# entn-at/tf-kaldi-speaker

Hardware: AMD Instinct MI355X
Metric: utterances/sec x-vector extraction (30-dim x 300-frame) (higher is better)
Workload: dtype f16+fp6-cross(f32-split); 1 GPU; tdnn x-vector (tdnn6_dense), statistics_pooling, 256 utt/GPU/step of 300 frames x 30 dims; batch_per_gpu=256, frames=300, node=tdnn6_dense, precision=f16f6, parallelism=utterance-shard x1, launch=stream launches

## Files before the change

tf-kaldi-speaker_amd/csrc/api_forward.hip:

```cpp
#include "xv_model.h"

using namespace xv;
using namespace xv::api;

namespace {

struct Run {
  xv_handle* h;
  const xv_plan* p;
  const float* feats;
  int feat_ld;
  float* out;
  char* ws;
  hipStream_t s;
  int f16;
  int B;
  const int32_t* off;
  char* raw(int64_t o) const { return o >= 0 ? ws + o : nullptr; }
  float* f32(int64_t o) const { return reinterpret_cast<float*>(raw(o)); }
  const float* in(int64_t o) const { return o == -2 ? feats : f32(o); }
  float* dst(const PlanStep& st) const { return st.out_off >= 0 ? f32(st.out_off) : out; }
  int* ovf() const { return static_cast<int*>(h->ovf_flag.p); }
};

// ... 25 lines not shown
  GemmArgs a{};
  a.X = r.in(st.in0_off);
  a.ldx = op.in0 == 0 ? r.feat_ld : L.cin;
  a.cin = L.cin; a.M = st.M; a.K = L.K(); a.N = L.cout;
  a.Wt = static_cast<const float*>(L.wt.p); a.Kpad = L.Kpad; a.Npad = L.Npad;
  const bool bn_stage = st.stage >= ST_BN;
  a.scale = (bn_stage || !L.has_bn) ? L.d_scale() : L.d_ones();
  a.shift = (bn_stage || !L.has_bn) ? L.d_shift() : L.d_bias();
  a.act = (st.stage == ST_ACT) ? L.act : ACT_NONE;
  a.alpha = (a.act == ACT_PRELU) ? L.d_alpha() : nullptr;
  a.rowmap = st.rowmap >= 0 ? static_cast<const int32_t*>(r.p->d_rowmaps.p) + r.p->rowmap_off[st.rowmap] : nullptr;
  a.Y = r.dst(st); a.ldy = L.cout;
  a.f16 = r.f16;
  a.slab3 = h->opt_slab3;
  a.ovf = r.ovf();
  a.sb_mul = std::ldexp(1.f, L.out_exp);
  if (L.mode == 1 || L.mode == 2 || L.mode == 3) {
    const int64_t Sin = h->values[op.in0].grid_S;
    a.a_pitch = (L.mode == 3 ? Sin : L.sw) * (int64_t)L.cin;
    a.a_off = L.mode == 1 ? (L.sw == 1 ? 0 : L.cin) : (L.mode == 2 ? (Sin + 1) * L.cin : L.cin);
    if (st.compact()) {
      a.arow = static_cast<const int32_t*>(r.p->d_rowmaps.p) + r.p->rowmap_off[st.arow];
      a.a_pitch = L.cin;
      a.a_off = L.mode == 1 ? 0 : (Sin + 1) * L.cin;
    }
    a.ntaps = L.mode == 1 ? 3 : 1;
    a.ktap = L.mode == 1 ? 3 * L.cin : (L.mode == 2 ? L.cin : L.Fin * L.cin);
    a.tap_stride = Sin * L.cin;
    a.cin = a.K;
  }
  if (op.in1 > 0) { a.R = r.in(st.in1_off); a.ldr = L.cout; }
  if (st.fuse_att == 1) {
    a.Y = nullptr;
    a.att_part = r.f32(st.out_off);
    a.att_ld = st.att_ld;
    a.att_heads = d.att_num_heads;
    a.att_q = static_cast<const float*>(h->query_eff.p);
  } else if (st.fuse_att == 2) {
    a.Y = nullptr;
    a.pool_part = r.f32(st.out_off);
    a.pool_row2utt = static_cast<const int32_t*>(r.p->d_row2utt.p);
    a.pool_slotbase = static_cast<const int32_t*>(r.p->d_slotbase.p);
    a.pool_w = r.f32(st.att_w_off);
    a.pool_heads = d.att_num_heads;
    a.pool_split = d.att_split_value;
    a.pool_dvh = d.att_split_value ? L.cout / d.att_num_heads : L.cout;
    a.pool_odim = h->pool_dim / 2;
  }
  if (st.fuse_pool) {
    a.Y = nullptr;
    a.pool_part = r.f32(st.out_off);
    a.pool_row2utt = static_cast<const int32_t*>(r.p->d_row2utt.p);
    a.pool_slotbase = static_cast<const int32_t*>(r.p->d_slotbase.p);
  }
  if (st.out_sb_off >= 0) {
    a.Ysb = r.raw(st.out_sb_off);
    a.ldsb = sb_ld(L.cout);
    if (st.out_off < 0 && !st.to_out) a.Y = nullptr;
  }
  return a;
}

int gemm_clear_border(const Run& r, const PlanStep& st, const Layer& L, const Value& vo) {
  xv_handle* h = r.h;
  const size_t head = (size_t)vo.grid_S + 1;
  const size_t rows0 = st.grid_cover && L.mode != 4 ? head : (st.grid_cover ? 0 : (size_t)st.rows_out + vo.grid_S);
  if (st.compact() || st.trows()) {
    XV_HIP(h, launch_grid_zero_border(r.p->dev_offsets(st.lvl_out), r.B, st.frames_out, vo.grid_F, vo.grid_S, L.cout / 4,
                                      sb_ld(L.cout) / 4, r.f32(st.out_off), r.raw(st.out_sb_off), r.s));
  } else {
    if (rows0 > 0) {
      if (st.out_off >= 0) XV_HIP(h, hipMemsetAsync(r.raw(st.out_off), 0, rows0 * L.cout * 4, r.s));
      if (st.out_sb_off >= 0) XV_HIP(h, hipMemsetAsync(r.raw(st.out_sb_off), 0, rows0 * sb_ld(L.cout) * 4, r.s));
    }
    const size_t tail = 2 * (size_t)vo.grid_S + 2;
    if (tail > (size_t)kSlackRows) return fail(h, XV_ERR_STATE, "grid pitch %d: the window overreach does not fit the slack", vo.grid_S);
    if (st.out_off >= 0) XV_HIP(h, hipMemsetAsync(r.f32(st.out_off) + (size_t)st.rows_out * L.cout, 0, tail * L.cout * 4, r.s));
    if (st.out_sb_off >= 0)
      XV_HIP(h, hipMemsetAsync(static_cast<char*>(r.raw(st.out_sb_off)) + (size_t)st.rows_out * sb_ld(L.cout) * 4, 0,
                               tail * sb_ld(L.cout) * 4, r.s));
  }
  return XV_OK;
}

int launch_conv0(const Run& r, const PlanStep& st, const Layer& L, const Value& vo, GemmArgs& a) {
  xv_handle* h = r.h;
  if (st.scratch_off < 0) return fail(h, XV_ERR_STATE, "conv0 has no scratch");
  a.cin = 32; a.K = 32;
  const bool direct = L.use_split && !st.to_out && st.stage == L.final_stage() && L.cout % 8 == 0 &&
                      (st.out_sb_off < 0 || L.cout % 32 == 0) && L.cout <= 256 && L.wdir.p;
  if (direct) {
    XV_HIP(h, launch_conv0_direct(r.feats, r.feat_ld, r.off, r.B, L.Fout, vo.grid_S, L.cout, st.M, static_cast<const float*>(L.wdir.p),
                                  L.act, L.d_alpha(), r.f32(st.out_off), r.raw(st.out_sb_off), sb_ld(L.cout), r.f16, r.ovf(),
                                  a.sb_mul, r.s));
  } else if (L.use_split) {
    XV_HIP(h, launch_im2col2d_sb(r.feats, r.feat_ld, r.off, r.B, L.Fout, vo.grid_S, st.M, r.raw(st.scratch_off), r.f16, r.ovf(), r.s));
    a.Xsb = r.raw(st.scratch_off); a.ldsbx = 32; a.Wsb = L.wsb.p; a.Wfr = L.wfr.p;
    XV_HIP(h, launch_gemm_bf16x3(a, r.s));
  } else {
    XV_HIP(h, launch_im2col2d_f32(r.feats, r.feat_ld, r.off, r.B, L.Fout, vo.grid_S, st.M, r.f32(st.scratch_off), r.s));
    a.X = r.f32(st.scratch_off); a.ldx = 32;
    XV_HIP(h, launch_gemm_f32(a, true, r.s));
  }
  return XV_OK;
}

// ... 319 lines not shown
```

tf-kaldi-speaker_amd/csrc/api_plan.hip:

```cpp
#include "xv_arena.h"
#include "xv_model.h"

using namespace xv;
using namespace xv::api;

namespace {

constexpr size_t kPoolMaxBuffers = 96, kPoolMaxBytes = (size_t)1 << 30;

hipError_t pool_take(xv_handle* h, size_t bytes, DevBuf& out) {
  out = DevBuf();
  if (bytes == 0) return hipSuccess;
  {
    std::lock_guard<std::mutex> lk(h->pool_mu);
    int best = -1;
    for (size_t i = 0; i < h->pool.size(); ++i)
      if (h->pool[i].bytes >= bytes && h->pool[i].bytes <= 4 * bytes + 4096 &&
          (best < 0 || h->pool[i].bytes < h->pool[best].bytes))
        best = (int)i;
    if (best >= 0) {
      out = h->pool[best];
      h->pool_bytes -= out.bytes;
      h->pool.erase(h->pool.begin() + best);
      return hipSuccess;
// ... 33 lines not shown
  BatchShape& sh = *out;
  sh.B = batch;
  for (int b = 0; b < batch; ++b) {
    const int64_t len = (int64_t)frame_offsets[b + 1] - frame_offsets[b];
    if (len <= need_ctx)
      return fail(h, XV_ERR_TOO_SHORT, "utterance %d has %lld frames; node '%s' needs more than %d", b, (long long)len,
                  h->nodes[node_id].name.c_str(), need_ctx);
    if (len != (int64_t)frame_offsets[1] - frame_offsets[0]) sh.uniform = false;
  }
  const int64_t F0 = frame_offsets[batch];
  if (F0 > (int64_t)1 << 30) return fail(h, XV_ERR_INVALID, "batch of %lld frames is too large for 32-bit row indices", (long long)F0);
  for (const Value& v : h->values) sh.max_level = std::max(sh.max_level, v.tlevel);
  for (int64_t& f : sh.Fl) f = F0;
  sh.lvl[0].assign(frame_offsets, frame_offsets + batch + 1);
  for (int k = 1; k <= sh.max_level && k < 4; ++k) {
    sh.lvl[k].resize(batch + 1);
    sh.lvl[k][0] = 0;
    for (int b = 0; b < batch; ++b) sh.lvl[k][b + 1] = sh.lvl[k][b] + (sh.lvl[k - 1][b + 1] - sh.lvl[k - 1][b] + 1) / 2;
    sh.Fl[k] = sh.lvl[k][batch];
  }
  return XV_OK;
}

std::vector<int> producers(const xv_handle* h) {
  std::vector<int> producer(h->values.size(), -1);
  for (size_t i = 0; i < h->ops.size(); ++i) producer[h->ops[i].out] = (int)i;
  return producer;
}

std::vector<int> plan_order(const xv_handle* h, int target_op, const std::vector<int>& producer) {
  std::vector<char> need(h->ops.size(), 0);
  std::vector<int> stack{target_op};
  while (!stack.empty()) {
    const int o = stack.back();
    stack.pop_back();
    if (need[o]) continue;
    need[o] = 1;
    for (int in : {h->ops[o].in0, h->ops[o].in1})
      if (in > 0 && producer[in] >= 0) stack.push_back(producer[in]);
  }
  std::vector<int> order;
  for (size_t i = 0; i < h->ops.size(); ++i) if (need[i]) order.push_back((int)i);
  return order;
}

struct Fusion {
  int key_prod = -1;
  int val_prod = -1;
  int att_pool_value = -1;
  int fused_value = -1;
  int slot_value = -1;
  std::vector<int> order;
  std::vector<int32_t> slotbase;
  int64_t pool_slots = 0;
};

int readers_of(const xv_handle* h, const std::vector<int>& order, int v) {
  int n = 0;
  for (int o : order)
    if (h->ops[o].in0 == v || h->ops[o].in1 == v) ++n;
  return n;
}

int att_fusable(const xv_handle* h, const std::vector<int>& order, const std::vector<int>& producer, int target_op, int v) {
  if (v <= 0 || producer[v] < 0 || producer[v] == target_op) return -1;
  const Op& prod = h->ops[producer[v]];
  if (prod.kind != OP_GEMM || prod.in1 > 0 || readers_of(h, order, v) != 1) return -1;
  const Layer& L = h->layers[prod.layer];
  return (L.use_split && !L.im2col && L.mode == 0 && L.w == 1 && (L.cout & 3) == 0) ? producer[v] : -1;
}

Fusion plan_fusion(const xv_handle* h, int target_op, const std::vector<int>& producer, std::vector<int> order, const BatchShape& sh) {
  Fusion f;
  if (h->opt_att_fusion && h->desc.pooling_type == XV_POOL_SELF_ATTENTION && h->desc.att_num_heads <= 8) {
    int softmax_op = -1, pool_op = -1;
    for (int o : order) {
      if (h->ops[o].kind == OP_ATT_SCORES) f.key_prod = att_fusable(h, order, producer, target_op, h->ops[o].in0);
      if (h->ops[o].kind == OP_ATT_SOFTMAX) softmax_op = o;
      if (h->ops[o].kind == OP_ATT_POOL) pool_op = o;
    }
    if (pool_op >= 0 && softmax_op >= 0) {
      const int H = h->desc.att_num_heads, dv = h->att_dv;
      const bool heads_ok = H == 1 || !h->desc.att_split_value || (dv / H) % 32 == 0;
      const int vp = heads_ok ? att_fusable(h, order, producer, target_op, h->ops[pool_op].in0) : -1;
      if (vp >= 0) {
        f.val_prod = vp;
        f.att_pool_value = h->ops[pool_op].in0;
        order.erase(std::find(order.begin(), order.end(), vp));
        order.insert(std::find(order.begin(), order.end(), pool_op), vp);
      }
    }
  }
  for (int o : order) {
    const Op& op = h->ops[o];
    if (op.kind != OP_STAT_POOL || op.in0 <= 0 || producer[op.in0] < 0) continue;
    const Op& prod = h->ops[producer[op.in0]];
    if (prod.kind != OP_GEMM || producer[op.in0] == target_op) continue;
    const Layer& L = h->layers[prod.layer];
    if (readers_of(h, order, op.in0) == 1 && L.w == 1 && (L.cout & 3) == 0 && h->opt_pool_fusion) f.fused_value = op.in0;
  }
  f.slot_value = f.fused_value >= 0 ? f.fused_value : f.att_pool_value;
  if (f.slot_value >= 0) {
    const int ctx = h->values[f.slot_value].ctx;
    const std::vector<int32_t>& so = sh.lvl[h->values[f.slot_value].tlevel];
    f.slotbase.resize(sh.B);
    for (int b = 0; b < sh.B; ++b) {
      const int r0 = so[b] - b * ctx, r1 = so[b + 1] - (b + 1) * ctx;
      const int t0 = r0 >> 6, t1 = (r1 - 1) >> 6;
      f.slotbase[b] = (int32_t)(f.pool_slots - t0);
      f.pool_slots += t1 - t0 + 1;
    }
  }
  f.order = std::move(order);
  return f;
}

struct PlanCtx {
  const xv_handle* h;
  const Node& node;
  const BatchShape& sh;
  const Fusion& fu;
  int64_t rows(int v) const { return value_rows(h, v, sh.Fl, sh.B); }
};

struct RowMaps {
  std::vector<int64_t> off;
  int64_t elems = 0;
  int add(int64_t n) { off.push_back(elems); elems += n; return (int)off.size() - 1; }
};

struct Placement {
  Arena arena;
  std::vector<int64_t> off, size, off_sb, size_sb;
  std::vector<char> want_f32, want_sb;
  std::vector<int> last_use;
  void free_value(int v) {
    if (size[v] > 0) { arena.release(off[v], size[v]); size[v] = 0; }
    if (size_sb[v] > 0) { arena.release(off_sb[v], size_sb[v]); size_sb[v] = 0; }
  }
};

Placement make_placement(const xv_handle* h, const std::vector<int>& order) {
  const size_t nv = h->values.size();
  Placement pl;
  pl.off.assign(nv, -1); pl.off_sb.assign(nv, -1);
  pl.size.assign(nv, 0); pl.size_sb.assign(nv, 0);
  pl.want_f32.assign(nv, 0); pl.want_sb.assign(nv, 0);
  pl.last_use.assign(nv, -1);
  for (size_t s = 0; s < order.size(); ++s) {
    const Op& op = h->ops[order[s]];
    const bool split_in = op.kind == OP_GEMM && h->layers[op.layer].use_split;
    if (op.in0 > 0) (split_in ? pl.want_sb : pl.want_f32)[op.in0] = 1;
    if (op.in1 > 0) pl.want_f32[op.in1] = 1;
    for (int in : {op.in0, op.in1})
      if (in > 0) pl.last_use[in] = (int)s;
  }
  return pl;
}

void gemm_form(const PlanCtx& c, const Op& op, const Layer& L, PlanStep& st, RowMaps& rm) {
  const xv_handle* h = c.h;
  const int64_t padded_rows = c.sh.Fl[st.lvl_in] + 2 * (int64_t)c.sh.B;
  const bool grid = L.mode == 1 || L.mode == 2;
// ... 259 lines not shown
  const Layer& L = h->layers[op.layer];
  const int B = p->info.batch;
  const Value& vi = h->values[op.in0];
  const Value& vo = h->values[op.out];
  const int32_t* doff = p->dev_offsets(st.lvl_in);
  int32_t* maps = static_cast<int32_t*>(p->d_rowmaps.p);
  int32_t* rm = maps + p->rowmap_off[st.rowmap];
  switch (st.form) {
    case FORM_ROWS: return launch_build_rowmap(doff, B, vi.ctx, L.w, rm, st.M, s);
    case FORM_TROWS: return launch_build_rowmap_trows(doff, B, vo.grid_S, rm, st.M, s);
    case FORM_COMPACT:
      return launch_build_rowmap_grid_compact(doff, p->dev_offsets(st.lvl_out), B, vi.grid_S, vo.grid_S, L.Fout, L.sw, L.st,
                                              L.mode == 1 ? 3 : 1, maps + p->rowmap_off[st.arow], rm, st.M, align_up(st.M, 128), s);
    case FORM_GRID:
      if (L.st == 2)
        return launch_build_rowmap_grid_ts(doff, p->dev_offsets(st.lvl_out), B, vi.grid_S / L.sw, L.Fout, vo.grid_S,
                                           L.mode == 1 ? 3 : 1, rm, st.M, s);
      return launch_build_rowmap_grid(doff, B, vi.grid_S / L.sw, L.Fout, vo.grid_S, st.grid_cover ? 1 : 0, rm, st.M, s);
    case FORM_CONV5: return launch_build_rowmap_rows(doff, B, rm, st.M, s);
    default: return launch_build_rowmap_interior(doff, B, L.Fout, vo.grid_S, rm, st.M, s);
  }
}

hipError_t upload_index_arrays(xv_plan* p, const BatchShape& sh, int64_t rowmap_elems, int slot_value, hipStream_t s, const char** what) {
  xv_handle* h = p->h;
  const size_t nb = (size_t)(sh.B + 1) * 4;
  hipError_t e = hipSuccess;
  DeviceGuard g(h->device);
  *what = "hipMalloc(offsets)";
  if ((e = pool_take(h, nb, p->d_offsets)) != hipSuccess) return e;
  *what = "hipMemcpyAsync(offsets)";
  if ((e = hipMemcpyAsync(p->d_offsets.p, p->lvl_offsets[0].data(), nb, hipMemcpyHostToDevice, s)) != hipSuccess) return e;
  for (int k = 1; k <= sh.max_level && k < 4; ++k) {
    *what = "hipMalloc(level offsets)";
    if ((e = pool_take(h, nb, p->d_lvl[k])) != hipSuccess) return e;
    *what = "hipMemcpyAsync(level offsets)";
    if ((e = hipMemcpyAsync(p->d_lvl[k].p, p->lvl_offsets[k].data(), nb, hipMemcpyHostToDevice, s)) != hipSuccess) return e;
  }
  if (rowmap_elems > 0) {
    *what = "hipMalloc(rowmaps)";
    if ((e = pool_take(h, (size_t)rowmap_elems * 4, p->d_rowmaps)) != hipSuccess) return e;
    *what = "build_rowmap";
    for (const PlanStep& st : p->steps)
      if (st.rowmap >= 0 && (e = build_rowmap(p, st, s)) != hipSuccess) return e;
  }
  if (slot_value >= 0) {
    const int64_t rows = value_rows(h, slot_value, sh.Fl, sh.B);
    *what = "hipMalloc(row2utt)";
    if ((e = pool_take(h, (size_t)rows * 4, p->d_row2utt)) != hipSuccess) return e;
    *what = "hipMalloc(slotbase)";
    if ((e = pool_take(h, (size_t)sh.B * 4, p->d_slotbase)) != hipSuccess) return e;
    *what = "hipMemcpyAsync(slotbase)";
    if ((e = hipMemcpyAsync(p->d_slotbase.p, p->offsets_slotbase.data(), (size_t)sh.B * 4, hipMemcpyHostToDevice, s)) != hipSuccess) return e;
    *what = "build_row2utt";
    e = launch_build_row2utt(p->dev_offsets(h->values[slot_value].tlevel), sh.B, h->values[slot_value].ctx,
                             static_cast<int32_t*>(p->d_row2utt.p), (int)rows, s);
  }
  return e;
}

}

extern "C" {

int xv_plan_create(xv_handle* h, const int32_t* frame_offsets, int batch, int node_id, void* stream, xv_plan** out) {
  if (!h) return fail(nullptr, XV_ERR_INVALID, "xv_plan_create: null handle");
  if (!out || !frame_offsets) return fail(h, XV_ERR_INVALID, "xv_plan_create: null argument");
  *out = nullptr;
  if (!h->finalized) return fail(h, XV_ERR_STATE, "xv_plan_create before xv_finalize");
  if (batch < 1) return fail(h, XV_ERR_INVALID, "xv_plan_create: batch %d < 1", batch);
  if (node_id < 0 || node_id >= (int)h->nodes.size()) return fail(h, XV_ERR_INVALID, "xv_plan_create: bad node id %d", node_id);
  const Node& node = h->nodes[node_id];
  BatchShape sh;
  if (const int rc = plan_shape(h, frame_offsets, batch, node_id, &sh)) return rc;
  if (node.att_weights && !sh.uniform)
    return fail(h, XV_ERR_INVALID, "attention_weights [b,h,l] needs utterances of equal length");
  const std::vector<int> producer = producers(h);
  const Fusion fu = plan_fusion(h, node.op, producer, plan_order(h, node.op, producer), sh);

  xv_plan* p = new (std::nothrow) xv_plan();
  if (!p) return fail(h, XV_ERR_HIP, "out of host memory");
  p->h = h;
  for (int k = 0; k <= sh.max_level && k < 4; ++k) p->lvl_offsets[k] = sh.lvl[k];
  p->pool_slots = fu.pool_slots;
  p->offsets_slotbase = fu.slotbase;

  const PlanCtx ctx{h, node, sh, fu};
  Placement pl = make_placement(h, fu.order);
  RowMaps rm;
  int64_t total_flops = 0;
  for (size_t s = 0; s < fu.order.size(); ++s) {
    p->steps.push_back(plan_step(ctx, s, p->steps, pl, rm));
    total_flops += p->steps.back().flops;
  }
  p->rowmap_off = rm.off;
  for (size_t i = 0; i < p->steps.size(); ++i)
    if (p->steps[i].flops > p->steps[p->dominant_step].flops) p->dominant_step = (int)i;
  chain_two_unit(h, p->steps);
  p->info = plan_output_info(h, node_id, sh, total_flops, pl.arena.top());

  const char* what = "";
  const hipError_t e = upload_index_arrays(p, sh, rm.elems, fu.slot_value, static_cast<hipStream_t>(stream), &what);
  if (e != hipSuccess) {
    const int rc = fail(h, XV_ERR_HIP, "%s failed: %s", what, hipGetErrorString(e));
    xv_plan_destroy(p);
    return rc;
  }
  *out = p;
  return XV_OK;
}

int xv_plan_query(const xv_plan* p, xv_plan_info* info) {
  if (!p || !info) return XV_ERR_INVALID;
  *info = p->info;
  return XV_OK;
}

void xv_plan_destroy(xv_plan* p) {
  if (!p) return;
  {
    DeviceGuard g(p->h->device);
    pool_give(p->h, p->d_offsets);
    for (int k = 1; k < 4; ++k) pool_give(p->h, p->d_lvl[k]);
    pool_give(p->h, p->d_rowmaps);
    pool_give(p->h, p->d_row2utt);
    pool_give(p->h, p->d_slotbase);
  }
  delete p;
}

}
```

tf-kaldi-speaker_amd/csrc/gemm_bf16x3.hip:

```cpp
#include <cstdlib>
#include <mutex>

#include "xv_f6.h"

namespace xv {

namespace {
constexpr int BM = 128, BN = 128;
constexpr int DROW = 128;
constexpr int DA_ROWS = 136;
constexpr int DA_BYTES = DA_ROWS * DROW;
typedef __attribute__((address_space(3))) void* lptr_t;
}

#define XV_GLD(dst, ptr, OFF) asm volatile("global_load_dwordx4 %0, %1, off offset:" #OFF : "=v"(dst) : "v"(ptr))
#define XV_WAIT4(N, ra, rb, rc, rd) asm volatile("s_waitcnt vmcnt(%4)" : "+v"(ra), "+v"(rb), "+v"(rc), "+v"(rd) : "n"(N))


__device__ __forceinline__ void tile_of_block(int id, int nMt, int nNt, int& mt, int& nt) {
  const int tile = xcd_remap(id, nMt * nNt);
  mt = tile / nNt;
  nt = tile - mt * nNt;
}

// ... 203 lines not shown
      koff_issue += 128;
    }
  };
  if (passive) {
    dma_slab(0, 0);
    advance();
    dma_slab(1 < nsteps ? koff_issue : 0, 1);
    advance();
    asm volatile("s_waitcnt vmcnt(0)" ::: "memory");
    __syncthreads();
    for (int s = 0, buf = 2; s < nsteps; ++s) {
      dma_slab(s + 2 < nsteps ? koff_issue : 0, buf);
      buf = buf == 2 ? 0 : buf + 1;
      asm volatile("s_waitcnt vmcnt(4)" ::: "memory");
      __syncthreads();
      advance();
    }
    asm volatile("s_waitcnt vmcnt(0)" ::: "memory");
    __syncthreads();
    return;
  }
  bf16x8 W0[4], W1[4], W2[4];
  {
    const char* q0 = Wg;
    const char* q1 = Wg + (int64_t)(1 < nsteps ? 1 : 0) * 4096;
    XV_GLD(W0[0], q0, 0); XV_GLD(W0[1], q0, 1024); XV_GLD(W0[2], q0, 2048); XV_GLD(W0[3], q0, 3072);
    XV_GLD(W1[0], q1, 0); XV_GLD(W1[1], q1, 1024); XV_GLD(W1[2], q1, 2048); XV_GLD(W1[3], q1, 3072);
  }
  dma_slab(0, 0);
  advance();
  dma_slab(1 < nsteps ? koff_issue : 0, 1);
  advance();
  asm volatile("s_waitcnt vmcnt(0)" ::: "memory");
  __syncthreads();

  XV_EPI_STAMP(p, 1);
  const int aswz = (c16 >> 1) & 7;
  const int off_hi = (g4 ^ aswz) << 4, off_lo = ((4 + g4) ^ aswz) << 4;
  auto step = [&](int s, int buf, bf16x8 (&Wc)[4], bf16x8 (&Wn)[4]) __attribute__((always_inline)) {
    const char* q = Wg + (int64_t)(s + 2 < nsteps ? s + 2 : 0) * 4096;
    const char* ab = As + buf * DA_BYTES + c16 * DROW;
    k_step<F16, 13>(acc, Wc, Wn, q, ab, off_hi, off_lo, [&]() __attribute__((always_inline)) {
      dma_slab(s + 2 < nsteps ? koff_issue : 0, buf == 0 ? 2 : buf - 1);
    });
    asm volatile("s_waitcnt vmcnt(12)" ::: "memory");
    __syncthreads();
    advance();
  };
  for (int s = 0; s < nsteps; s += 3) {
    step(s, 0, W0, W2);
    if (s + 1 < nsteps) step(s + 1, 1, W1, W0);
    if (s + 2 < nsteps) step(s + 2, 2, W2, W1);
  }
  const int lane_e = end_k_loop(p, lane);
  if constexpr (EPI == 3) store_wave_tile_n32_f6(p, acc, m0, n0 + wave * 32, lane_e, wave, smem3);
  else if constexpr (EPI != 0) store_wave_tile_n32_att<EPI>(p, acc, m0, n0 + wave * 32, lane_e, wave, smem3);
  else store_wave_tile_n32<64, F16>(p, acc, m0, n0 + wv * 32, lane_e, wave, smem3);
  XV_EPI_STAMP(p, 3);
}

template <int EPI = 0, bool F16 = false, bool GATHER = false>
__global__ __launch_bounds__(256, 3) void gemm_bf16x3_w1p3_kernel(GemmArgs p, int nMt, int nNt) {
  extern __shared__ __attribute__((aligned(16))) char smem3[];
  int mt, nt;
  tile_of_block(blockIdx.x, nMt, nNt, mt, nt);
  w1p3_tile<EPI, F16, GATHER>(p, mt * BM, nt * BN, smem3);
}

template <int NPS, int EPI = 0, bool F16 = false>
__global__ __launch_bounds__(256, 3) void gemm_bf16x3_w14p2_kernel(GemmArgs p, int nMt, int nNt, int w, int S) {
  extern __shared__ __attribute__((aligned(16))) char smem3[];
  int mt, nt, cb_begin = 0, cb_end = (p.Kpad >> 5) / w;
  constexpr bool kSlices = EPI == 0 || EPI == 3;
  const bool slice = kSlices && (int)blockIdx.x >= nMt * nNt;
  if (slice) {
    const int id = blockIdx.x - nMt * nNt;
    const int split = id % S, tile = id / S;
    mt = nMt + tile / nNt;
    nt = tile % nNt;
    const int per = cb_end / S;
    cb_begin = split * per;
    cb_end = cb_begin + per;
    p.Y = p.partial + ((int64_t)split * p.tail_mt - nMt) * (int64_t)BM * p.Npad;
    p.ldy = p.Npad;
    if (EPI == 0) {
      p.raw = 1;
      p.act = ACT_NONE;
      p.alpha = nullptr;
      p.N = p.Npad;
      p.M = (nMt + p.tail_mt) * BM;
      p.Ysb = nullptr;
      p.rowmap = nullptr;
      p.R = nullptr;
      p.pool_part = nullptr;
    }
  } else {
    tile_of_block(blockIdx.x, nMt, nNt, mt, nt);
  }
  w14p2_tile<NPS, EPI, F16>(p, mt * BM, nt * BN, w, smem3, cb_begin, cb_end, slice);
}

__global__ void bf16x3_tail_reduce_kernel(GemmArgs p, int mt0, int S) {
  const int quads = p.Npad >> 2;
  const int64_t rows = (int64_t)p.tail_mt * BM;
  const int64_t total = rows * quads;
  for (int64_t i = (int64_t)blockIdx.x * blockDim.x + threadIdx.x; i < total; i += (int64_t)gridDim.x * blockDim.x) {
    const int64_t r = i / quads;
    const int n = (int)(i - r * quads) * 4;
// ... 77 lines not shown
  if (tiles <= slots || r == 0 || r > slots / 4) return 0;
  const int mt = (r + nNt - 1) / nNt;
  int S = 0;
  for (int c = 8; c >= 2; c >>= 1)
    if (ncb % c == 0 && ncb / c >= 2 && (ncb / c) % cb_quant == 0 && mt * nNt * c <= 256) { S = c; break; }
  if (S == 0) return 0;
  *tail_mt = mt;
  *splits = S;
  return (int64_t)S * mt * BM * Npad * (int64_t)sizeof(float);
}

namespace {
template <int NPS, int EPI>
auto w14p2_kernel(bool f16) {
  if constexpr (EPI == 3) return gemm_bf16x3_w14p2_kernel<NPS, 3, true>;
  else return f16 ? gemm_bf16x3_w14p2_kernel<NPS, EPI, true> : gemm_bf16x3_w14p2_kernel<NPS, EPI, false>;
}
template <int EPI, bool GATHER = false>
auto w1p3_kernel(bool f16) {
  if constexpr (EPI == 3) return gemm_bf16x3_w1p3_kernel<3, true, GATHER>;
  else return f16 ? gemm_bf16x3_w1p3_kernel<EPI, true, GATHER> : gemm_bf16x3_w1p3_kernel<EPI, false, GATHER>;
}
}

hipError_t launch_gemm_bf16x3(const GemmArgs& a_in, hipStream_t s) {
  if (a_in.M <= 0) return hipSuccess;
  GemmArgs a = a_in;
  trace_arm(a, s);
  static std::mutex init_mu;
  static bool attr_set[64] = {};
  const size_t smemw32 = (size_t)2 * DA_BYTES;
  const size_t smemw1p3 = (size_t)3 * DA_BYTES;
  int dev = 0;
  if (hipGetDevice(&dev) != hipSuccess) dev = 0;
  {
    std::lock_guard<std::mutex> init_lock(init_mu);
    if (!attr_set[dev & 63]) {
      const void* kernels[] = {
          reinterpret_cast<const void*>(gemm_bf16x3_w14p2_kernel<1, 0, false>), reinterpret_cast<const void*>(gemm_bf16x3_w14p2_kernel<4, 0, false>),
          reinterpret_cast<const void*>(gemm_bf16x3_w14p2_kernel<4, 1, false>), reinterpret_cast<const void*>(gemm_bf16x3_w14p2_kernel<4, 2, false>),
          reinterpret_cast<const void*>(gemm_bf16x3_w14p2_kernel<1, 0, true>), reinterpret_cast<const void*>(gemm_bf16x3_w14p2_kernel<4, 0, true>),
          reinterpret_cast<const void*>(gemm_bf16x3_w14p2_kernel<4, 1, true>), reinterpret_cast<const void*>(gemm_bf16x3_w14p2_kernel<4, 2, true>),
          reinterpret_cast<const void*>(gemm_bf16x3_w14p2_kernel<1, 3, true>), reinterpret_cast<const void*>(gemm_bf16x3_w14p2_kernel<4, 3, true>)};
      hipError_t r = hipSuccess;
      for (const void* k : kernels) {
        r = hipFuncSetAttribute(k, hipFuncAttributeMaxDynamicSharedMemorySize, (int)smemw32);
        if (r != hipSuccess) return r;
      }
      const void* kernels3[] = {
          reinterpret_cast<const void*>(gemm_bf16x3_w1p3_kernel<0, false>), reinterpret_cast<const void*>(gemm_bf16x3_w1p3_kernel<0, true>),
          reinterpret_cast<const void*>(gemm_bf16x3_w1p3_kernel<1, false>), reinterpret_cast<const void*>(gemm_bf16x3_w1p3_kernel<1, true>),
          reinterpret_cast<const void*>(gemm_bf16x3_w1p3_kernel<2, false>), reinterpret_cast<const void*>(gemm_bf16x3_w1p3_kernel<2, true>),
          reinterpret_cast<const void*>(gemm_bf16x3_w1p3_kernel<0, false, true>), reinterpret_cast<const void*>(gemm_bf16x3_w1p3_kernel<0, true, true>),
          reinterpret_cast<const void*>(gemm_bf16x3_w1p3_kernel<3, true>), reinterpret_cast<const void*>(gemm_bf16x3_w1p3_kernel<3, true, true>)};
      for (const void* k : kernels3) {
        r = hipFuncSetAttribute(k, hipFuncAttributeMaxDynamicSharedMemorySize, (int)smemw1p3);
        if (r != hipSuccess) return r;
      }
      attr_set[dev & 63] = true;
    }
  }
  const int w = a.K / a.cin > 0 && a.ldsbx == a.cin ? a.K / a.cin : 1;
  const bool taps_ok = w <= 9 && (a.Kpad >> 5) % w == 0;
  const int nNt = a.Npad / BN, nMt = (a.M + BM - 1) / BM;
  if (!taps_ok) return hipErrorInvalidValue;
  const dim3 block(256);
  if (a.att_part || a.pool_w) {
    if (w != 1 || a.rowmap || a.a_pitch || a.R || (a.N & 3) || (a.pool_w && !a.pool_part)) return hipErrorInvalidValue;
    const dim3 grid(nMt * nNt);
    if (!a.slab3) {
      if (a.att_part) hipLaunchKernelGGL((w14p2_kernel<4, 1>(a.f16)), grid, block, smemw32, s, a, nMt, nNt, w, 0);
      else            hipLaunchKernelGGL((w14p2_kernel<4, 2>(a.f16)), grid, block, smemw32, s, a, nMt, nNt, w, 0);
    } else {
      if (a.att_part) hipLaunchKernelGGL((w1p3_kernel<1>(a.f16)), grid, block, smemw1p3, s, a, nMt, nNt);
      else            hipLaunchKernelGGL((w1p3_kernel<2>(a.f16)), grid, block, smemw1p3, s, a, nMt, nNt);
    }
    return hipGetLastError();
  }
  const bool tail = a.tail_mt > 0 && a.ksplit > 1 && a.partial && !a.a_pitch && !a.pool_part && !a.R && !a.raw &&
                    a.tail_mt < nMt && (a.N & 3) == 0;
  const int nMain = tail ? nMt - a.tail_mt : nMt;
  const dim3 grid(nMain * nNt);
  trace_grid(a, grid.x);
  if (a.arow) {
    if (w != 1 || tail || !a.a_pitch || a.pool_part) return hipErrorInvalidValue;
    if (a.ysb_f6 && (!a.f16 || !a.Ysb || a.Y || a.R)) return hipErrorInvalidValue;
    if (a.ysb_f6) hipLaunchKernelGGL((w1p3_kernel<3, true>(a.f16)), grid, block, smemw1p3, s, a, nMain, nNt);
    else          hipLaunchKernelGGL((w1p3_kernel<0, true>(a.f16)), grid, block, smemw1p3, s, a, nMain, nNt);
    return hipGetLastError();
  }
  if (a.ysb_f6 && (!a.f16 || (w > 1 && w < 5) || !a.Ysb || a.Y || a.R || a.pool_part)) return hipErrorInvalidValue;
  if (w == 1 && !tail && a.slab3) {
    if (a.ysb_f6) hipLaunchKernelGGL((w1p3_kernel<3>(a.f16)), grid, block, smemw1p3, s, a, nMain, nNt);
    else          hipLaunchKernelGGL((w1p3_kernel<0>(a.f16)), grid, block, smemw1p3, s, a, nMain, nNt);
    return hipGetLastError();
  }
  const int S = tail ? a.ksplit : 0;
  const dim3 grid2(nMain * nNt + (tail ? a.tail_mt * nNt * a.ksplit : 0));
  if (a.ysb_f6) {
    if (w >= 5) hipLaunchKernelGGL((w14p2_kernel<1, 3>(a.f16)), grid2, block, smemw32, s, a, nMain, nNt, w, S);
    else        hipLaunchKernelGGL((w14p2_kernel<4, 3>(a.f16)), grid2, block, smemw32, s, a, nMain, nNt, w, S);
  } else {
    if (w >= 5) hipLaunchKernelGGL((w14p2_kernel<1, 0>(a.f16)), grid2, block, smemw32, s, a, nMain, nNt, w, S);
    else        hipLaunchKernelGGL((w14p2_kernel<4, 0>(a.f16)), grid2, block, smemw32, s, a, nMain, nNt, w, S);
  }
  const hipError_t e = hipGetLastError();
  if (e != hipSuccess || !tail) return e;
  if (a.ysb_f6) return launch_f6v2_tail_reduce(a, nMain, s);
  const int64_t total = (int64_t)a.tail_mt * BM * (a.Npad >> 2);
  hipLaunchKernelGGL(bf16x3_tail_reduce_kernel, dim3((unsigned)((total + 255) / 256)), block, 0, s, a, nMain, a.ksplit);
  return hipGetLastError();
}

}
```

tf-kaldi-speaker_amd/csrc/xv_epilogue.h:

```cpp
#pragma once
#include "xv_kernels.h"

namespace xv {

typedef float f32x16 __attribute__((ext_vector_type(16)));
typedef float f32x4 __attribute__((ext_vector_type(4)));
typedef short bf16x8 __attribute__((ext_vector_type(8)));

__device__ __forceinline__ float apply_act(float v, int act, float alpha) {
  switch (act) {
    case ACT_RELU: return fmaxf(v, 0.0f);
    case ACT_LRELU: return fmaxf(v, kLreluAlpha * v);
    case ACT_PRELU: return fmaxf(v, 0.0f) + alpha * (v - fabsf(v)) * 0.5f;
    case ACT_TANH: return tanhf(v);
    default: return v;
  }
}

#ifdef XV_GEMM_TRACE
#define XV_EPI_STAMP(p, i)                                                                                          \
  do {                                                                                                              \
    if ((p).trace && threadIdx.x == 0) (p).trace[(int64_t)blockIdx.x * 8 + (i)] = (long long)__builtin_amdgcn_s_memrealtime(); \
  } while (0)
#define XV_EPI_DRAIN() asm volatile("s_waitcnt vmcnt(0) lgkmcnt(0)" ::: "memory")
// ... 562 lines not shown
          s1 = groups_sum(s1);
          const f32x4 mu = s1 * (1.0f / 64.0f);
          f32x4 m2 = z;
#pragma unroll 4
          for (int k = 0; k < 8; ++k) {
            const f32x4 d = row4(k * 8 + rrow) - mu;
            m2 += d * d;
          }
          m2 = groups_sum(m2);
          if (nok && rrow == 0) {
            const int64_t slot = (int64_t)p.pool_slotbase[u_first] + tile64;
            *reinterpret_cast<f32x4*>(p.pool_part + (slot * 2) * p.N + n) = s1;
            *reinterpret_cast<f32x4*>(p.pool_part + (slot * 2 + 1) * p.N + n) = m2;
          }
        } else {
          int r = 0;
          while (r < 64) {
            const int b = __builtin_amdgcn_readlane(my_utt, r);
            const unsigned long long same = __ballot(my_utt == b) >> r;
            const int re = r + (~same ? __builtin_ctzll(~same) : 64 - r);
            if (b >= 0) {
              f32x4 s1 = z;
              for (int t0 = r & ~7; t0 < re; t0 += 8) {
                const int t = t0 + rrow;
                if (t >= r && t < re) s1 += row4(t);
              }
              s1 = groups_sum(s1);
              const f32x4 mu = s1 / (float)(re - r);
              f32x4 m2 = z;
              for (int t0 = r & ~7; t0 < re; t0 += 8) {
                const int t = t0 + rrow;
                if (t >= r && t < re) {
                  const f32x4 d = row4(t) - mu;
                  m2 += d * d;
                }
              }
              m2 = groups_sum(m2);
              if (nok && rrow == 0) {
                const int64_t slot = (int64_t)p.pool_slotbase[b] + tile64;
                *reinterpret_cast<f32x4*>(p.pool_part + (slot * 2) * p.N + n) = s1;
                *reinterpret_cast<f32x4*>(p.pool_part + (slot * 2 + 1) * p.N + n) = m2;
              }
            }
            r = re;
          }
        }
      }
      if (ps == 0) XV_EPI_STAMP(p, 7);
      wave_lds_sync();
    }
  }
}

__device__ __forceinline__ float slot_inverse(float s0) { return s0 >= 1.17549435e-38f ? 1.0f / s0 : 0.f; }

template <int ACT, int FORM>
__device__ __forceinline__ void store_wave_tile_n32_att_impl(const GemmArgs& p, const f32x4 (&acc)[8][2], int mbase, int nbase,
                                                             int lane, int wave, char* lds) {
  const int c16 = lane & 15, g4 = lane >> 4;
  const f32x4 z = {0.f, 0.f, 0.f, 0.f};
  f32x4 sc[2], sh[2];
#pragma unroll
  for (int ct = 0; ct < 2; ++ct) {
    const int n4 = nbase + 16 * ct + 4 * g4;
    const bool ok = n4 < p.N;
    sc[ct] = ok ? *reinterpret_cast<const f32x4*>(p.scale + n4) : z;
    sh[ct] = ok ? *reinterpret_cast<const f32x4*>(p.shift + n4) : z;
  }
  auto value4 = [&](const f32x4& t, int ct) -> f32x4 {
    f32x4 al = z;
    if (ACT < 0 && p.alpha && nbase + 16 * ct + 4 * g4 < p.N) al = *reinterpret_cast<const f32x4*>(p.alpha + nbase + 16 * ct + 4 * g4);
    f32x4 v;
#pragma unroll
    for (int i = 0; i < 4; ++i) v[i] = apply_act(fmaf(t[i], sc[ct][i], sh[ct][i]), ACT < 0 ? p.act : ACT, al[i]);
    return v;
  };
  if constexpr (FORM == 1) {
    const int blk = nbase >> 5;
#pragma unroll
    for (int ft = 0; ft < 8; ++ft) {
      f32x4 v[2];
#pragma unroll
      for (int ct = 0; ct < 2; ++ct) v[ct] = value4(acc[ft][ct], ct);
      const int m = mbase + ft * 16 + c16;
      for (int hd = 0; hd < p.att_heads; ++hd) {
        const float* qp = p.att_q + (int64_t)hd * p.Npad + nbase + 4 * g4;
        float s = 0.f;
#pragma unroll
        for (int ct = 0; ct < 2; ++ct) {
          const f32x4 qv = *reinterpret_cast<const f32x4*>(qp + 16 * ct);
#pragma unroll
          for (int i = 0; i < 4; ++i) s = fmaf(v[ct][i], qv[i], s);
        }
        s += __shfl_xor(s, 16, 64);
        s += __shfl_xor(s, 32, 64);
        if (g4 == 0 && m < p.M) p.att_part[((int64_t)blk * p.att_heads + hd) * p.att_ld + m] = s;
      }
    }
    return;
  } else {
  char* scratch = lds + wave * (64 * 128);
  const int rrow = lane >> 3, rchunk = lane & 7;
  const int n = nbase + rchunk * 4;
  const bool nok = n < p.N;
  const int H = p.pool_heads;
  const int hd0 = p.pool_split ? min(nbase / p.pool_dvh, H - 1) : 0;
// ... 154 lines not shown
```

tf-kaldi-speaker_amd/csrc/xv_kernels.h:

```cpp
#pragma once
#include <hip/hip_runtime.h>
#include <stdint.h>

#include <string>

#include "../../include/xvec_hip.h"

namespace xv {

enum Act : int { ACT_NONE = 0, ACT_RELU = 1, ACT_LRELU = 2, ACT_PRELU = 3, ACT_TANH = 4 };

constexpr float kLreluAlpha = 0.2f;
constexpr int kFlagWords = 8, kUttSmallWord = 4, kFeatMaxSlots = 32768;
constexpr int kUttMaxSlots = 32768;
constexpr int kFlagBufWords = kFlagWords + kFeatMaxSlots + kUttMaxSlots;
constexpr float kVarFloor = 1e-12f;

struct GemmArgs {
  const float* X;
  int64_t ldx;
  int cin;
  int M;
  int K;
  int N;
  const float* Wt;
  int Kpad;
  int Npad;
  const float* scale;
  const float* shift;
  const float* alpha;
  int act;
  const int32_t* rowmap;
  float* Y;
  int64_t ldy;
  const void* Xsb;
  int64_t ldsbx;
  void* Ysb;
  int ldsb;
  const void* Wsb;
  const void* Wfr = nullptr;
  const void* Wx6 = nullptr;
  int ysb_f6 = 0;
  int slab3 = 1;
  int* ovf = nullptr;
  int nbin = 0;
  int64_t bin_x_bytes = 0;
  float sb_mul = 1.f;
  int f16 = 0;
  long long* trace = nullptr;
  int ksplit;
  int raw;
  float* partial;
  int tail_mt = 0;
  float* pool_part;
  const int32_t* pool_row2utt;
  const int32_t* pool_slotbase;
  int64_t a_pitch;
  int64_t a_off;
  int64_t tap_stride;
  int ntaps;
  int ktap;
  const int32_t* arow;
  const float* R;
  int64_t ldr;
  const float* att_q = nullptr;
  float* att_part = nullptr;
  int64_t att_ld = 0;
  int att_heads = 0;
  const float* pool_w = nullptr;
  int pool_heads = 0;
  int pool_split = 0;
  int pool_dvh = 0;
  int pool_odim = 0;
};

hipError_t launch_gemm_f32(const GemmArgs& a, bool aligned, hipStream_t s);

int gemm_f32_ksplit(int M, int Kpad, int Npad);

int64_t gemm_bf16x3_tail_plan(int M, int Kpad, int Npad, int w, int* tail_mt, int* splits, int cb_quant = 1);

hipError_t launch_im2col_sb(const float* x, int64_t ldx, int cin, int w, int64_t rows, void* out_sb, int ldsb, int f16,
                            int* ovf, hipStream_t s);

bool feat_stage_sb_ok(int ldsb, int batch);
hipError_t launch_feat_stage_sb(const float* x, int64_t ldx, int cin, const int32_t* offsets_dev, int batch, int max_len,
                                void* out_sb, int ldsb, int f16, int* flags, hipStream_t s);

hipError_t launch_gemm_bf16x3(const GemmArgs& a, hipStream_t s);
hipError_t launch_gemm_f16f6(const GemmArgs& a, hipStream_t s);
hipError_t launch_f6v2_tail_reduce(const GemmArgs& a, int nMain, hipStream_t s);
hipError_t launch_f6_from_sb(const void* sb, void* out, int64_t rows, int nblk, hipStream_t s);

hipError_t launch_build_rowmap(const int32_t* off0, int B, int ctx_in, int w, int32_t* rowmap, int M,
                               hipStream_t s);

hipError_t launch_stat_pool(const float* x, int64_t ldx, int C, const int32_t* off0, int B, int ctx,
                            float* out, int64_t ldo, hipStream_t s);

hipError_t launch_build_row2utt(const int32_t* off0, int B, int ctx, int32_t* row2utt, int M, hipStream_t s);
hipError_t launch_pool_finalize(const float* part, int C, const int32_t* off0, int B, int ctx,
                                const int32_t* slotbase, float* out, int64_t ldo, hipStream_t s);

hipError_t launch_build_rowmap_grid(const int32_t* off0, int B, int rows_per_t, int Fout, int So, int cover, int32_t* rowmap,
                                    int64_t M, hipStream_t s);
hipError_t launch_build_rowmap_grid_ts(const int32_t* off_in, const int32_t* off_out, int B, int rows_per_t, int Fout, int So,
                                       int ktime, int32_t* rowmap, int64_t M, hipStream_t s);
hipError_t launch_build_rowmap_grid_compact(const int32_t* off_in, const int32_t* off_out, int B, int Sin, int So, int Fout,
                                            int sw, int st, int ktime, int32_t* arow, int32_t* rowmap, int64_t M, int64_t Mpad,
                                            hipStream_t s);
hipError_t launch_grid_zero_border(const int32_t* off0, int B, int64_t frames, int F, int S, int chunks_y, int chunks_sb,
                                   float* y, void* ysb, hipStream_t s);
hipError_t launch_build_rowmap_rows(const int32_t* off0, int B, int32_t* rowmap, int64_t M, hipStream_t s);
hipError_t launch_build_rowmap_trows(const int32_t* off0, int B, int So, int32_t* rowmap, int64_t M, hipStream_t s);
hipError_t launch_build_rowmap_interior(const int32_t* off0, int B, int F, int S, int32_t* rowmap, int64_t M, hipStream_t s);
hipError_t launch_im2col2d_sb(const float* x, int64_t ldx, const int32_t* off0, int B, int F, int S, int64_t P, void* out_sb,
                              int f16, int* ovf, hipStream_t s);
hipError_t launch_im2col2d_f32(const float* x, int64_t ldx, const int32_t* off0, int B, int F, int S, int64_t P, float* out,
                               hipStream_t s);
hipError_t launch_conv0_direct(const float* x, int64_t ldx, const int32_t* off0, int B, int F, int S, int C, int64_t P,
                               const float* wdir, int act, const float* alpha, float* y, void* ysb, int ldsb, int f16, int* ovf,
                               float sb_mul, hipStream_t s);
hipError_t launch_grid_maxpool3x3(const float* x, const int32_t* off0, int B, int F, int S, int C, int64_t P, float* y,
                                  void* ysb, int ldsb, int f16, int* ovf, float sb_mul, hipStream_t s);
hipError_t launch_grid_unpad_n(const float* grid, const int32_t* off0, int B, int F, int S, int C, int64_t frames, float* out,
                               hipStream_t s);
// ... 146 lines not shown
```

tf-kaldi-speaker_amd/csrc/xv_model.h:

```cpp
#pragma once
#include <hip/hip_runtime.h>

#include <algorithm>
#include <cmath>
#include <cstdio>
#include <cstring>
#include <map>
#include <mutex>
#include <string>
#include <vector>

#include "../../include/xvec_hip.h"
#include "xv_kernels.h"

namespace xv {
namespace api {

constexpr int kSlackRows = 512;
constexpr int kAlign = 256;

struct DevBuf {
  void* p = nullptr;
  size_t bytes = 0;
  hipError_t alloc(size_t n) {
// ... 152 lines not shown
};

struct PlanStep {
  int op = -1;
  int stage = -1;
  bool to_out = false;
  int64_t out_off = -1;
  int64_t out_sb_off = -1;
  int64_t in0_off = -1, in1_off = -1;
  int64_t in0_sb_off = -1;
  int64_t rows_in = 0, rows_out = 0;
  int M = 0;
  int form = FORM_ROWS;
  bool trows() const { return form == FORM_TROWS; }
  bool compact() const { return form == FORM_COMPACT; }
  int rowmap = -1;
  int64_t scratch_off = -1;
  int64_t scratch2_off = -1;
  int ksplit = 1;
  int tail_mt = 0;
  bool fuse_pool = false;
  int lvl_in = 0, lvl_out = 0;
  int64_t frames_out = 0;
  bool grid_cover = false;
  bool out_f6 = false;
  bool in_f6 = false;
  int arow = -1;
  int fuse_att = 0;
  int64_t att_w_off = -1;
  int64_t att_s0_off = -1;
  int64_t att_ld = 0;
  bool unpad_to_out = false;
  int64_t flops = 0, bytes = 0;
};

}
}

struct xv_plan {
  xv_handle* h = nullptr;
  xv_plan_info info{};
  std::vector<int32_t> offsets_slotbase;
  xv::api::DevBuf d_offsets;
  std::vector<int32_t> lvl_offsets[4];
  xv::api::DevBuf d_lvl[4];
  const int32_t* dev_offsets(int level) const {
    return static_cast<const int32_t*>(level > 0 ? d_lvl[level].p : d_offsets.p);
  }
  xv::api::DevBuf d_rowmaps;
  std::vector<int64_t> rowmap_off;
  std::vector<xv::api::PlanStep> steps;
  xv::api::DevBuf d_row2utt;
  xv::api::DevBuf d_slotbase;
  int64_t pool_slots = 0;
  int dominant_step = 0;
};

namespace xv {
namespace api {

int fail(xv_handle* h, int code, const char* fmt, ...);

#define XV_HIP(h, expr)                                                                              \
  do {                                                                                               \
    hipError_t _e = (expr);                                                                          \
    if (_e != hipSuccess)                                                                            \
      return fail((h), XV_ERR_HIP, "%s failed: %s (%s:%d)", #expr, hipGetErrorString(_e), __FILE__,  \
                  __LINE__);                                                                         \
  } while (0)

inline int64_t align_up(int64_t v, int64_t a) { return (v + a - 1) / a * a; }

inline int act_of(const xv_model_desc& d) {
  return d.relu_type == XV_ACT_PRELU ? ACT_PRELU : (d.relu_type == XV_ACT_LRELU ? ACT_LRELU : ACT_RELU);
}

inline int64_t value_rows(const xv_handle* h, int vid, const int64_t* Fl, int B) {
  const Value& v = h->values[vid];
  if (v.grid_F > 0) return (Fl[v.tlevel] + 2 * (int64_t)B) * v.grid_S;
  return v.frame_level ? Fl[v.tlevel] - (int64_t)B * v.ctx : B;
}

inline int64_t value_bytes(const xv_handle* h, int vid, const int64_t* Fl, int B) {
  const Value& v = h->values[vid];
  return align_up((value_rows(h, vid, Fl, B) + kSlackRows) * (int64_t)v.cols * 4, kAlign);
}

inline int sb_ld(int cols) { return (int)align_up(cols, 32); }

inline int64_t value_sb_bytes(const xv_handle* h, int vid, const int64_t* Fl, int B) {
  const Value& v = h->values[vid];
  return align_up((value_rows(h, vid, Fl, B) + kSlackRows) * (int64_t)sb_ld(v.cols) * 4, kAlign);
}

}
}
```

Before: 227,000 utterances/s.

## Add specialized pool-fused GEMM epilogue driven by precomputed per-tile segment descriptors

Builds a host-side table at plan time that gives, for each 64-row tile, up to two utterance slots and their row counts, and uploads it to the device. A new GEMM epilogue variant (EPI=4) loads these descriptors through scalar constant loads. Tiles fully inside one utterance reduce sum and M2 with DPP row reductions and skip the LDS round trip and the per-row utterance lookup. Mixed tiles still use the LDS path. This adds a kernel instantiation and a small device buffer per plan, and tiles touching more than two utterances get zeroed descriptors.

```diff
diff --git a/tf-kaldi-speaker_amd/csrc/api_forward.hip b/tf-kaldi-speaker_amd/csrc/api_forward.hip
--- a/tf-kaldi-speaker_amd/csrc/api_forward.hip
+++ b/tf-kaldi-speaker_amd/csrc/api_forward.hip
@@ -101,6 +101,7 @@
     a.pool_part = r.f32(st.out_off);
     a.pool_row2utt = static_cast<const int32_t*>(r.p->d_row2utt.p);
     a.pool_slotbase = static_cast<const int32_t*>(r.p->d_slotbase.p);
+    if (st.M == r.p->pool_pass_rows) a.pool_pass = static_cast<const int32_t*>(r.p->d_pool_pass.p);
   }
   if (st.out_sb_off >= 0) {
     a.Ysb = r.raw(st.out_sb_off);
diff --git a/tf-kaldi-speaker_amd/csrc/api_plan.hip b/tf-kaldi-speaker_amd/csrc/api_plan.hip
--- a/tf-kaldi-speaker_amd/csrc/api_plan.hip
+++ b/tf-kaldi-speaker_amd/csrc/api_plan.hip
@@ -109,6 +109,8 @@
   int slot_value = -1;
   std::vector<int> order;
   std::vector<int32_t> slotbase;
+  std::vector<int32_t> pool_pass;
+  int64_t pool_pass_rows = 0;
   int64_t pool_slots = 0;
 };
 
@@ -166,6 +168,23 @@
       const int t0 = r0 >> 6, t1 = (r1 - 1) >> 6;
       f.slotbase[b] = (int32_t)(f.pool_slots - t0);
       f.pool_slots += t1 - t0 + 1;
+    }
+    const int64_t rows = so[sh.B] - (int64_t)sh.B * ctx, npass = (rows + 127) / 128 * 2;
+    f.pool_pass_rows = rows;
+    f.pool_pass.assign((size_t)npass * 4, 0);
+    int b = 0;
+    for (int64_t t = 0; t < npass; ++t) {
+      const int64_t lo = t * 64, hi = std::min(lo + 64, rows);
+      int32_t* d = &f.pool_pass[(size_t)t * 4];
+      d[0] = d[2] = -1;
+      while (b < sh.B && so[b + 1] - (int64_t)(b + 1) * ctx <= lo) ++b;
+      int nseg = 0;
+      for (int u = b; u < sh.B && so[u] - (int64_t)u * ctx < hi; ++u, ++nseg) {
+        if (nseg >= 2) continue;
+        d[2 * nseg] = (int32_t)(f.slotbase[u] + t);
+        d[2 * nseg + 1] = (int32_t)(std::min<int64_t>(so[u + 1] - (int64_t)(u + 1) * ctx, hi) - std::max<int64_t>(so[u] - (int64_t)u * ctx, lo));
+      }
+      if (nseg > 2) d[0] = d[1] = d[2] = d[3] = 0;
     }
   }
   f.order = std::move(order);
@@ -531,6 +550,12 @@
     if ((e = pool_take(h, (size_t)sh.B * 4, p->d_slotbase)) != hipSuccess) return e;
     *what = "hipMemcpyAsync(slotbase)";
     if ((e = hipMemcpyAsync(p->d_slotbase.p, p->offsets_slotbase.data(), (size_t)sh.B * 4, hipMemcpyHostToDevice, s)) != hipSuccess) return e;
+    if (!p->pool_pass.empty()) {
+      *what = "hipMalloc(pool passes)";
+      if ((e = pool_take(h, p->pool_pass.size() * 4, p->d_pool_pass)) != hipSuccess) return e;
+      *what = "hipMemcpyAsync(pool passes)";
+      if ((e = hipMemcpyAsync(p->d_pool_pass.p, p->pool_pass.data(), p->pool_pass.size() * 4, hipMemcpyHostToDevice, s)) != hipSuccess) return e;
+    }
     *what = "build_row2utt";
     e = launch_build_row2utt(p->dev_offsets(h->values[slot_value].tlevel), sh.B, h->values[slot_value].ctx,
                              static_cast<int32_t*>(p->d_row2utt.p), (int)rows, s);
@@ -563,6 +588,8 @@
   for (int k = 0; k <= sh.max_level && k < 4; ++k) p->lvl_offsets[k] = sh.lvl[k];
   p->pool_slots = fu.pool_slots;
   p->offsets_slotbase = fu.slotbase;
+  p->pool_pass = fu.pool_pass;
+  p->pool_pass_rows = fu.pool_pass_rows;
 
   const PlanCtx ctx{h, node, sh, fu};
   Placement pl = make_placement(h, fu.order);
@@ -604,6 +631,7 @@
     pool_give(p->h, p->d_rowmaps);
     pool_give(p->h, p->d_row2utt);
     pool_give(p->h, p->d_slotbase);
+    pool_give(p->h, p->d_pool_pass);
   }
   delete p;
 }
diff --git a/tf-kaldi-speaker_amd/csrc/gemm_bf16x3.hip b/tf-kaldi-speaker_amd/csrc/gemm_bf16x3.hip
--- a/tf-kaldi-speaker_amd/csrc/gemm_bf16x3.hip
+++ b/tf-kaldi-speaker_amd/csrc/gemm_bf16x3.hip
@@ -279,8 +279,18 @@
     if (s + 1 < nsteps) step(s + 1, 1, W1, W0);
     if (s + 2 < nsteps) step(s + 2, 2, W2, W1);
   }
+  int pd[2][4];
+  if constexpr (EPI == 4) {
+    int m0e = m0;
+    asm volatile("" : "+s"(m0e));
+    typedef const __attribute__((address_space(4))) int32_t* cptr_t;
+    const cptr_t dq = (cptr_t)(uintptr_t)(p.pool_pass + (int64_t)(m0e >> 6) * 4);
+#pragma unroll
+    for (int i = 0; i < 8; ++i) pd[i >> 2][i & 3] = dq[i];
+  }
   const int lane_e = end_k_loop(p, lane);
   if constexpr (EPI == 3) store_wave_tile_n32_f6(p, acc, m0, n0 + wave * 32, lane_e, wave, smem3);
+  else if constexpr (EPI == 4) store_wave_tile_n32_pool(p, acc, m0, n0 + wave * 32, lane_e, wave, smem3, pd);
   else if constexpr (EPI != 0) store_wave_tile_n32_att<EPI>(p, acc, m0, n0 + wave * 32, lane_e, wave, smem3);
   else store_wave_tile_n32<64, F16>(p, acc, m0, n0 + wv * 32, lane_e, wave, smem3);
   XV_EPI_STAMP(p, 3);
@@ -464,7 +474,8 @@
           reinterpret_cast<const void*>(gemm_bf16x3_w1p3_kernel<1, false>), reinterpret_cast<const void*>(gemm_bf16x3_w1p3_kernel<1, true>),
           reinterpret_cast<const void*>(gemm_bf16x3_w1p3_kernel<2, false>), reinterpret_cast<const void*>(gemm_bf16x3_w1p3_kernel<2, true>),
           reinterpret_cast<const void*>(gemm_bf16x3_w1p3_kernel<0, false, true>), reinterpret_cast<const void*>(gemm_bf16x3_w1p3_kernel<0, true, true>),
-          reinterpret_cast<const void*>(gemm_bf16x3_w1p3_kernel<3, true>), reinterpret_cast<const void*>(gemm_bf16x3_w1p3_kernel<3, true, true>)};
+          reinterpret_cast<const void*>(gemm_bf16x3_w1p3_kernel<3, true>), reinterpret_cast<const void*>(gemm_bf16x3_w1p3_kernel<3, true, true>),
+          reinterpret_cast<const void*>(gemm_bf16x3_w1p3_kernel<4, false>), reinterpret_cast<const void*>(gemm_bf16x3_w1p3_kernel<4, true>)};
       for (const void* k : kernels3) {
         r = hipFuncSetAttribute(k, hipFuncAttributeMaxDynamicSharedMemorySize, (int)smemw1p3);
         if (r != hipSuccess) return r;
@@ -503,8 +514,10 @@
   }
   if (a.ysb_f6 && (!a.f16 || (w > 1 && w < 5) || !a.Ysb || a.Y || a.R || a.pool_part)) return hipErrorInvalidValue;
   if (w == 1 && !tail && a.slab3) {
-    if (a.ysb_f6) hipLaunchKernelGGL((w1p3_kernel<3>(a.f16)), grid, block, smemw1p3, s, a, nMain, nNt);
-    else          hipLaunchKernelGGL((w1p3_kernel<0>(a.f16)), grid, block, smemw1p3, s, a, nMain, nNt);
+    const bool pool_epi = a.pool_part && a.pool_pass && !a.Y && !a.Ysb && !a.R && !a.rowmap && !a.raw && (a.N & 3) == 0;
+    if (a.ysb_f6)      hipLaunchKernelGGL((w1p3_kernel<3>(a.f16)), grid, block, smemw1p3, s, a, nMain, nNt);
+    else if (pool_epi) hipLaunchKernelGGL((w1p3_kernel<4>(a.f16)), grid, block, smemw1p3, s, a, nMain, nNt);
+    else               hipLaunchKernelGGL((w1p3_kernel<0>(a.f16)), grid, block, smemw1p3, s, a, nMain, nNt);
     return hipGetLastError();
   }
   const int S = tail ? a.ksplit : 0;
diff --git a/tf-kaldi-speaker_amd/csrc/xv_epilogue.h b/tf-kaldi-speaker_amd/csrc/xv_epilogue.h
--- a/tf-kaldi-speaker_amd/csrc/xv_epilogue.h
+++ b/tf-kaldi-speaker_amd/csrc/xv_epilogue.h
@@ -638,6 +638,134 @@
   }
 }
 
+template <int ACT>
+__device__ __forceinline__ void store_wave_tile_n32_pool_impl(const GemmArgs& p, const f32x4 (&acc)[8][2], int mbase, int nbase,
+                                                              int lane, int wave, char* lds, const int (&pd)[2][4]) {
+  const int c16 = lane & 15, g4 = lane >> 4;
+  const f32x4 z = {0.f, 0.f, 0.f, 0.f};
+  f32x4 sc[2], sh[2];
+#pragma unroll
+  for (int ct = 0; ct < 2; ++ct) {
+    const int n4 = nbase + 16 * ct + 4 * g4;
+    const bool ok = n4 < p.N;
+    sc[ct] = ok ? *reinterpret_cast<const f32x4*>(p.scale + n4) : z;
+    sh[ct] = ok ? *reinterpret_cast<const f32x4*>(p.shift + n4) : z;
+  }
+  auto value4 = [&](const f32x4& t, int ct) -> f32x4 {
+    f32x4 al = z;
+    if (ACT < 0 && p.alpha && nbase + 16 * ct + 4 * g4 < p.N) al = *reinterpret_cast<const f32x4*>(p.alpha + nbase + 16 * ct + 4 * g4);
+    f32x4 v;
+#pragma unroll
+    for (int i = 0; i < 4; ++i) v[i] = apply_act(fmaf(t[i], sc[ct][i], sh[ct][i]), ACT < 0 ? p.act : ACT, al[i]);
+    return v;
+  };
+  auto row_sum = [&](float x) -> float {
+    x += __builtin_bit_cast(float, __builtin_amdgcn_update_dpp(0, __builtin_bit_cast(int, x), 0xB1, 0xF, 0xF, true));
+    x += __builtin_bit_cast(float, __builtin_amdgcn_update_dpp(0, __builtin_bit_cast(int, x), 0x4E, 0xF, 0xF, true));
+    x += __builtin_bit_cast(float, __builtin_amdgcn_update_dpp(0, __builtin_bit_cast(int, x), 0x141, 0xF, 0xF, true));
+    x += __builtin_bit_cast(float, __builtin_amdgcn_update_dpp(0, __builtin_bit_cast(int, x), 0x140, 0xF, 0xF, true));
+    return x;
+  };
+  auto store_slot = [&](int64_t slot, int ct, const f32x4& s1, const f32x4& m2) {
+    const int nn = nbase + 16 * ct + 4 * g4;
+    if (c16 == 0 && nn < p.N) {
+      *reinterpret_cast<f32x4*>(p.pool_part + (slot * 2) * p.N + nn) = s1;
+      *reinterpret_cast<f32x4*>(p.pool_part + (slot * 2 + 1) * p.N + nn) = m2;
+    }
+  };
+  auto pass = [&](auto pass_index) __attribute__((always_inline)) {
+    constexpr int ps = decltype(pass_index)::value;
+    const int slot0 = pd[ps][0], n0 = pd[ps][1];
+    if (n0 == 64) {
+#pragma unroll
+      for (int ct = 0; ct < 2; ++ct) {
+        f32x4 s1 = z;
+#pragma unroll
+        for (int fl = 0; fl < 4; ++fl) s1 += value4(acc[ps * 4 + fl][ct], ct);
+#pragma unroll
+        for (int i = 0; i < 4; ++i) s1[i] = row_sum(s1[i]);
+        const f32x4 mu = s1 * (1.0f / 64.0f);
+        f32x4 m2 = z;
+#pragma unroll
+        for (int fl = 0; fl < 4; ++fl) {
+          const f32x4 d = value4(acc[ps * 4 + fl][ct], ct) - mu;
+          m2 += d * d;
+        }
+#pragma unroll
+        for (int i = 0; i < 4; ++i) m2[i] = row_sum(m2[i]);
+        store_slot(slot0, ct, s1, m2);
+      }
+    } else if (slot0 >= 0) {
+      char* scratch = lds + wave * (64 * 128);
+      const int rrow = lane >> 3, rchunk = lane & 7;
+      const int n = nbase + rchunk * 4;
+      const int mb = mbase + ps * 64;
+#pragma unroll
+      for (int fl = 0; fl < 4; ++fl)
+#pragma unroll
+        for (int ct = 0; ct < 2; ++ct) {
+          const int row = fl * 16 + c16;
+          *reinterpret_cast<f32x4*>(scratch + row * 128 + (((4 * ct + g4) ^ swz8(row)) << 4)) = value4(acc[ps * 4 + fl][ct], ct);
+        }
+      wave_lds_sync();
+      const int my_utt = (mb + lane < p.M) ? p.pool_row2utt[mb + lane] : -1;
+      auto row4 = [&](int t) -> f32x4 {
+        return *reinterpret_cast<const f32x4*>(scratch + t * 128 + ((rchunk ^ swz8(t)) << 4));
+      };
+      auto groups_sum = [&](f32x4 v) -> f32x4 {
+#pragma unroll
+        for (int i = 0; i < 4; ++i) {
+          v[i] += __shfl_xor(v[i], 8, 64);
+          v[i] += __shfl_xor(v[i], 16, 64);
+          v[i] += __shfl_xor(v[i], 32, 64);
+        }
+        return v;
+      };
+      int r = 0;
+      while (r < 64) {
+        const int b = __builtin_amdgcn_readlane(my_utt, r);
+        const unsigned long long same = __ballot(my_utt == b) >> r;
+        const int re = r + (~same ? __builtin_ctzll(~same) : 64 - r);
+        if (b >= 0) {
+          f32x4 s1 = z;
+          for (int t0 = r & ~7; t0 < re; t0 += 8) {
+            const int t = t0 + rrow;
+            if (t >= r && t < re) s1 += row4(t);
+          }
+          s1 = groups_sum(s1);
+          const f32x4 mu = s1 / (float)(re - r);
+          f32x4 m2 = z;
+          for (int t0 = r & ~7; t0 < re; t0 += 8) {
+            const int t = t0 + rrow;
+            if (t >= r && t < re) {
+              const f32x4 d = row4(t) - mu;
+              m2 += d * d;
+            }
+          }
+          m2 = groups_sum(m2);
+          if (n < p.N && rrow == 0) {
+            const int64_t slot = (int64_t)p.pool_slotbase[b] + (mb >> 6);
+            *reinterpret_cast<f32x4*>(p.pool_part + (slot * 2) * p.N + n) = s1;
+            *reinterpret_cast<f32x4*>(p.pool_part + (slot * 2 + 1) * p.N + n) = m2;
+          }
+        }
+        r = re;
+      }
+      wave_lds_sync();
+    }
+  };
+  pass(std::integral_constant<int, 0>());
+  pass(std::integral_constant<int, 1>());
+}
+
+__device__ __forceinline__ void store_wave_tile_n32_pool(const GemmArgs& p, const f32x4 (&acc)[8][2], int mbase, int nbase,
+                                                         int lane, int wave, char* lds, const int (&pd)[2][4]) {
+  if (p.act == ACT_RELU)
+    store_wave_tile_n32_pool_impl<ACT_RELU>(p, acc, mbase, nbase, lane, wave, lds, pd);
+  else
+    store_wave_tile_n32_pool_impl<-1>(p, acc, mbase, nbase, lane, wave, lds, pd);
+}
+
 __device__ __forceinline__ float slot_inverse(float s0) { return s0 >= 1.17549435e-38f ? 1.0f / s0 : 0.f; }
 
 template <int ACT, int FORM>
diff --git a/tf-kaldi-speaker_amd/csrc/xv_kernels.h b/tf-kaldi-speaker_amd/csrc/xv_kernels.h
--- a/tf-kaldi-speaker_amd/csrc/xv_kernels.h
+++ b/tf-kaldi-speaker_amd/csrc/xv_kernels.h
@@ -72,6 +72,7 @@
   int pool_split = 0;
   int pool_dvh = 0;
   int pool_odim = 0;
+  const int32_t* pool_pass = nullptr;
 };
 
 hipError_t launch_gemm_f32(const GemmArgs& a, bool aligned, hipStream_t s);
diff --git a/tf-kaldi-speaker_amd/csrc/xv_model.h b/tf-kaldi-speaker_amd/csrc/xv_model.h
--- a/tf-kaldi-speaker_amd/csrc/xv_model.h
+++ b/tf-kaldi-speaker_amd/csrc/xv_model.h
@@ -228,6 +228,9 @@
   std::vector<xv::api::PlanStep> steps;
   xv::api::DevBuf d_row2utt;
   xv::api::DevBuf d_slotbase;
+  std::vector<int32_t> pool_pass;
+  xv::api::DevBuf d_pool_pass;
+  int64_t pool_pass_rows = 0;
   int64_t pool_slots = 0;
   int dominant_step = 0;
 };
```

After: 227,700 utterances/s (median of 6 runs). No clear change (+0.3%).
